# Orange-OpenSource/AIVC

Measured on AMD Instinct MI355X. Metric: encode+decode fps @1080p YUV420 (RA GOP32), higher is better.
Workload: dtype f32; 1 GPU; 1920x1080 8-bit YUV420, coding structure 1_GOP_32: one 128-frame clip = 4 intra-period units of 33 frames (132 coded frames, the last 4 repeat the last frame) encoded + decoded per step; synthetic random-init stand-in for model ms_ssim-4 (widths {'n2': 64, 'n': 128, 'c_y': 64, 'c_short': 64, 'c_z': 32, 'n_h': 128}), last analysis conv calibrated so that 6 (MOFNet) / 12 (CodecNet) of the 64 y featu; parallelism=single GPU

## Files before the change

aivc_amd/csrc/entropy.hip:

```cpp
#include <stdlib.h>
#include <string.h>

#include "common.h"

namespace aivc {

__device__ float balle_cdf_point(const float *P, float t) {
  const float *h0 = P, *h1 = P + 3, *h2 = P + 12, *h3 = P + 21;
  const float *b0 = P + 24, *b1 = P + 27, *b2 = P + 30, *b3 = P + 33;
  const float *a0 = P + 34, *a1 = P + 37, *a2 = P + 40;
  float v[3], nv[3];
#pragma unroll
  for (int r = 0; r < 3; ++r) {
    float x = t * aivc_softplusf_det(h0[r]);
    x = x + b0[r];
    v[r] = x + aivc_tanhf_det(a0[r]) * aivc_tanhf_det(x);
  }
#pragma unroll
  for (int l = 0; l < 2; ++l) {
    const float *hh = l == 0 ? h1 : h2;
    const float *bb = l == 0 ? b1 : b2;
    const float *aa = l == 0 ? a1 : a2;
#pragma unroll
    for (int r = 0; r < 3; ++r) {
      float acc = v[0] * aivc_softplusf_det(hh[0 * 3 + r]);
      acc = __builtin_fmaf(v[1], aivc_softplusf_det(hh[1 * 3 + r]), acc);
      acc = __builtin_fmaf(v[2], aivc_softplusf_det(hh[2 * 3 + r]), acc);
      const float x = acc + bb[r];
      nv[r] = x + aivc_tanhf_det(aa[r]) * aivc_tanhf_det(x);
    }
    v[0] = nv[0];
    v[1] = nv[1];
    v[2] = nv[2];
  }
  float acc = v[0] * aivc_softplusf_det(h3[0]);
  acc = __builtin_fmaf(v[1], aivc_softplusf_det(h3[1]), acc);
  acc = __builtin_fmaf(v[2], aivc_softplusf_det(h3[2]), acc);
  return aivc_sigmoidf_det(acc + b3[0]);
}

__global__ __launch_bounds__(256) void balle_cdf_table_kernel(const float *__restrict__ params, int c,
                                                              uint16_t *__restrict__ table,
                                                              float *__restrict__ cdf_f32) {
  const int gid = blockIdx.x * blockDim.x + threadIdx.x;
  if (gid >= c * AIVC_CDF_ROW) return;
  const int ch = gid / AIVC_CDF_ROW, k = gid % AIVC_CDF_ROW;
  if (k >= AIVC_LP) {
    table[gid] = 0;
    return;
  }
  const float cdf = balle_cdf_point(params + (size_t)ch * AIVC_BALLE_PARAMS, (float)k - 256.5f);
  if (cdf_f32) cdf_f32[(size_t)ch * AIVC_LP + k] = cdf;
  table[gid] = aivc_cdf_quant(cdf, k);
}

__global__ __launch_bounds__(256) void nonzero_maps_kernel(const int16_t *__restrict__ q, size_t npix, int c,
                                                           uint8_t *__restrict__ flags) {
  q += (size_t)blockIdx.y * npix * c;
  flags += (size_t)blockIdx.y * c;
  for (size_t i = (size_t)blockIdx.x * blockDim.x + threadIdx.x; i < npix * c; i += (size_t)gridDim.x * blockDim.x)
    if (q[i] != 0) flags[i % c] = 1;
}

__global__ __launch_bounds__(256) void laplace_cdf_rows_kernel(const float *__restrict__ sigma, size_t npix, int c,
                                                               aivc_map_list maps, uint16_t *__restrict__ rows) {
  constexpr int CHUNKS = AIVC_CDF_ROW / 8;
  const size_t gid = (size_t)blockIdx.x * blockDim.x + threadIdx.x;
  const size_t total = (size_t)maps.n_maps * npix * CHUNKS;
  if (gid >= total) return;
  const int chunk = (int)(gid % CHUNKS);
  const size_t pos = gid / CHUNKS;
  const int m = (int)(pos / npix);
  const size_t pix = pos % npix;
  const float s = sigma[pix * c + maps.idx[m]];
  uint32_t w[4];
#pragma unroll
  for (int j = 0; j < 4; ++j) {
    const int k0 = chunk * 8 + 2 * j, k1 = k0 + 1;
    const uint32_t lo = k0 < AIVC_LP ? aivc_laplace_cdf_u16(k0, s) : 0;
    const uint32_t hi = k1 < AIVC_LP ? aivc_laplace_cdf_u16(k1, s) : 0;
    w[j] = lo | (hi << 16);
  }
  *reinterpret_cast<uint4 *>(rows + pos * AIVC_CDF_ROW + chunk * 8) = make_uint4(w[0], w[1], w[2], w[3]);
}

using FrameTable = const aivc_frame_maps *__restrict__;
__device__ __forceinline__ const aivc_frame_maps &frame_of(FrameTable frames) { return frames[blockIdx.y]; }
__device__ __forceinline__ const aivc_frame_maps &frame_of(const aivc_frame_maps &fm) { return fm; }

constexpr int CDF_WIN0 = 224, CDF_WIN = 64;
template <class FRAMES>
__global__ __launch_bounds__(256) void laplace_cdf_windows_batch_kernel(const float *__restrict__ sigma, size_t npix, int c,
                                                                        const FRAMES frames, uint16_t *__restrict__ win,
                                                                        float *__restrict__ sigma_pos) {
  constexpr int CHUNKS = CDF_WIN / 8;
  const aivc_frame_maps &fm = frame_of(frames);
  const size_t gid = (size_t)blockIdx.x * blockDim.x + threadIdx.x;
  const size_t total = (size_t)fm.n_maps * npix;
  const size_t wv = gid >> 6;
  if ((wv / CHUNKS) * 64 >= total) return;
  const int lane = (int)(gid & 63), chunk = (int)(wv % CHUNKS);
  const size_t pos = (wv / CHUNKS) * 64 + (size_t)lane;
  const bool valid = pos < total;
  const float *sg = sigma + (size_t)blockIdx.y * npix * c;
  float s = 1.0f;
  if (valid) {
    const int m = (int)(pos / npix);
    const size_t pix = pos % npix;
    s = sg[pix * c + fm.idx[m]];
    if (chunk == 0) sigma_pos[fm.pos_off + pos] = s;
  }
  const int k0 = CDF_WIN0 + chunk * 8;
  uint32_t w[4];
  bool sat = false;
  if (chunk != CHUNKS / 2) {
    const float tmin = chunk < CHUNKS / 2 ? 256.5f - (float)(k0 + 7) : (float)k0 - 256.5f;
    const float b = s / 1.41421354f;
    sat = tmin / b > 17.5f;
  }
  if (__all(sat || !valid)) {
    const uint32_t base = chunk < CHUNKS / 2 ? 0u : 65023u;
#pragma unroll
    for (int j = 0; j < 4; ++j) {
      const uint32_t k = (uint32_t)(k0 + 2 * j);
      w[j] = ((base + k) & 0xFFFFu) | (((base + k + 1u) & 0xFFFFu) << 16);
    }
  } else {
#pragma unroll
    for (int j = 0; j < 4; ++j) {
      const int k = k0 + 2 * j;
      w[j] = (uint32_t)aivc_laplace_cdf_u16(k, s) | ((uint32_t)aivc_laplace_cdf_u16(k + 1, s) << 16);
    }
  }
  if (valid) *reinterpret_cast<uint4 *>(win + (fm.pos_off + pos) * CDF_WIN + chunk * 8) = make_uint4(w[0], w[1], w[2], w[3]);
}

template <class FRAMES>
__global__ __launch_bounds__(256) void laplace_bounds_batch_kernel(const float *__restrict__ sigma, const int16_t *__restrict__ q,
                                                                   size_t npix, int c, const FRAMES frames,
                                                                   uint32_t *__restrict__ bounds) {
  const aivc_frame_maps &fm = frame_of(frames);
  const size_t pos = (size_t)blockIdx.x * blockDim.x + threadIdx.x;
  if (pos >= (size_t)fm.n_maps * npix) return;
  const int ch = fm.idx[pos / npix];
  const size_t pix = pos % npix;
  const size_t o = ((size_t)blockIdx.y * npix + pix) * c + ch;
  const float s = sigma[o];
  const int sym = min(max((int)q[o] + AIVC_AC_MAX_VAL, 0), AIVC_MAX_SYMBOL);
  const uint32_t lo = aivc_laplace_cdf_u16(sym, s), hi = sym == AIVC_MAX_SYMBOL ? 0u : aivc_laplace_cdf_u16(sym + 1, s);
  bounds[fm.pos_off + pos] = lo | (hi << 16);
}

template <class FRAMES>
__global__ __launch_bounds__(256) void scatter_symbols_batch_kernel(const uint16_t *__restrict__ sym, size_t npix, int c,
                                                                    const FRAMES frames, int16_t *__restrict__ q, int vec) {
  __shared__ int16_t slot[AIVC_MAX_MAPS];
  const aivc_frame_maps &fm = frame_of(frames);
  for (int i = threadIdx.x; i < AIVC_MAX_MAPS; i += blockDim.x) slot[i] = -1;
  __syncthreads();
  for (int i = threadIdx.x; i < fm.n_maps; i += blockDim.x) slot[fm.idx[i]] = (int16_t)i;
  __syncthreads();
  const size_t gid = (size_t)blockIdx.x * blockDim.x + threadIdx.x;
  const int groups = (c + 7) / 8;
  if (gid >= npix * groups) return;
  const size_t pix = gid % npix;
  const int ch0 = (int)(gid / npix) * 8;
  const uint16_t *fs = sym + fm.pos_off;
  int16_t v[8];
#pragma unroll
  for (int e = 0; e < 8; ++e) {
    const int ch = ch0 + e;
    const int m = ch < c ? slot[ch] : -1;
    v[e] = m < 0 ? (int16_t)0 : (int16_t)((int)fs[(size_t)m * npix + pix] - AIVC_AC_MAX_VAL);
  }
  int16_t *dst = q + ((size_t)blockIdx.y * npix + pix) * c + ch0;
  if (vec) {
    uint4 o;
    o.x = (uint32_t)(uint16_t)v[0] | ((uint32_t)(uint16_t)v[1] << 16);
    o.y = (uint32_t)(uint16_t)v[2] | ((uint32_t)(uint16_t)v[3] << 16);
    o.z = (uint32_t)(uint16_t)v[4] | ((uint32_t)(uint16_t)v[5] << 16);
    o.w = (uint32_t)(uint16_t)v[6] | ((uint32_t)(uint16_t)v[7] << 16);
    *reinterpret_cast<uint4 *>(dst) = o;
  } else {
#pragma unroll
    for (int e = 0; e < 8; ++e)
      if (ch0 + e < c) dst[e] = v[e];
  }
}

__global__ __launch_bounds__(256) void table_bounds_batch_kernel(const uint16_t *__restrict__ table, const int16_t *__restrict__ q,
                                                                 size_t npix, int c, uint32_t *__restrict__ bounds) {
  const size_t pos = (size_t)blockIdx.x * blockDim.x + threadIdx.x;
  if (pos >= (size_t)c * npix) return;
  const int ch = (int)(pos / npix);
  const size_t pix = pos % npix;
  const int sym = min(max((int)q[((size_t)blockIdx.y * npix + pix) * c + ch] + AIVC_AC_MAX_VAL, 0), AIVC_MAX_SYMBOL);
  const uint16_t *row = table + (size_t)ch * AIVC_CDF_ROW;
  bounds[(size_t)blockIdx.y * c * npix + pos] = (uint32_t)row[sym] | (sym == AIVC_MAX_SYMBOL ? 0u : (uint32_t)row[sym + 1] << 16);
}

__device__ __forceinline__ uint32_t rl(uint32_t v, int lane) { return __builtin_amdgcn_readlane(v, lane); }

__device__ __forceinline__ uint32_t scaled(uint32_t e, uint32_t hl) {
  uint64_t r, carry;
  const uint64_t e64 = e;
  asm("v_mad_u64_u32 %0, %1, %2, %3, %4" : "=&v"(r), "=s"(carry) : "v"(e), "s"(hl), "v"(e64));
  uint32_t t = (uint32_t)(r >> 16);
  asm("" : "+v"(t));
  return t;
}

struct BitSink {
  uint32_t *out;
  uint32_t cap_words;
  uint32_t n_words;
  uint64_t acc;
  uint32_t nbits;
  uint32_t overflow;
  __device__ __forceinline__ void put(uint32_t bits, uint32_t nb) {
    acc = (acc << nb) | (uint64_t)bits;
    nbits += nb;
    if (nbits >= 32) {
      nbits -= 32;
      const uint32_t w = (uint32_t)(acc >> nbits);
      if (n_words < cap_words) out[n_words] = __builtin_bswap32(w);
      else overflow = 1;
      n_words++;
    }
  }
  __device__ __forceinline__ void put_run(uint32_t bit, uint32_t count) {
    while (count > 0) {
      const uint32_t r = count > 32 ? 32 : count;
      const uint32_t ones = r == 32 ? 0xFFFFFFFFu : ((1u << r) - 1u);
      put(bit ? ones : 0u, r);
      count -= r;
    }
  }
  __device__ __forceinline__ void finish() {
    if (nbits > 0) {
      const uint32_t w = (uint32_t)(acc << (32 - nbits));
      if (n_words < cap_words) out[n_words] = __builtin_bswap32(w);
      else overflow = 1;
    }
  }
};

__global__ __launch_bounds__(64) void range_encode_kernel(const uint32_t *__restrict__ bounds, aivc_rc_batch batch,
                                                          uint8_t *__restrict__ out, uint32_t *__restrict__ out_len) {
  const aivc_rc_stream st = batch.s[blockIdx.x];
  const int lane = threadIdx.x;
  __builtin_amdgcn_s_setprio(3);
  BitSink sink{reinterpret_cast<uint32_t *>(out + st.out_off), st.out_cap / 4, 0, 0, 0, 0};
  uint32_t low = 0, high = 0xFFFFFFFFu, pending = 0;
  const uint32_t *src = bounds + st.in_off;
  uint32_t nxt = lane < (int)st.n_sym ? src[lane] : 0u;
#pragma unroll 1
  for (uint32_t base = 0; base < st.n_sym; base += 64) {
    const uint32_t mine = nxt;
    nxt = (base + 64u + lane < st.n_sym) ? src[base + 64u + lane] : 0u;
    const uint32_t vlo = mine & 0xFFFFu, vhi = (mine >> 16) ? (mine >> 16) : 0x10000u;
    const uint32_t cnt = min(64u, st.n_sym - base);
#pragma unroll 1
    for (uint32_t j = 0; j < cnt; ++j) {
      const uint32_t hl = high - low;
      const uint32_t t_lo = rl(scaled(vlo, hl), (int)j), t_hi = rl(scaled(vhi, hl), (int)j);
      high = low + t_hi - 1u;
      low = low + t_lo;
      const uint32_t x = low ^ high;
      if ((int32_t)x >= 0) {
        const uint32_t n = (uint32_t)__builtin_clz(x | 1u);
        const uint32_t top = (uint32_t)(((uint64_t)low << n) >> 32);
        uint32_t bits = top, nb = n;
        if (pending != 0) {
          const uint32_t b0 = low >> 31;
          sink.put(b0, 1);
          sink.put_run(b0 ^ 1u, pending);
          pending = 0;
          nb = n - 1u;
          bits = top & ((1u << nb) - 1u);
        }
        sink.put(bits, nb);
        low <<= n;
        high = (high << n) | ~(0xFFFFFFFFu << n);
      }
      asm volatile("" : "+s"(high));
      const uint32_t yy = low & ~high;
      if (yy & 0x40000000u) {
        const uint32_t m = (uint32_t)__builtin_clz(~(yy << 1));
        pending += m;
        low = (low << m) & 0x7FFFFFFFu;
        high = (high << m) | 0x80000000u | ((1u << m) - 1u);
      }
    }
  }
  pending += 1;
  const uint32_t fb = low < 0x40000000u ? 0u : 1u;
  sink.put(fb, 1);
  sink.put_run(fb ^ 1u, pending);
  sink.finish();
  const uint32_t total = sink.n_words * 4u + (sink.nbits + 7u) / 8u;
  if (total > st.out_cap) sink.overflow = 1;
  if (lane == 0) out_len[blockIdx.x] = sink.overflow ? 0xFFFFFFFFu : total;
}

constexpr int ENC_CH = 32;

struct LanePacker {
  uint32_t *dst;
  uint32_t last_word;
  uint32_t widx;
  uint64_t acc;
  uint32_t nbits;
  __device__ __forceinline__ void push(uint32_t val, uint32_t len) {
    acc = (acc << len) | (uint64_t)val;
    nbits += len;
    dst[min(widx, last_word)] = __builtin_bswap32((uint32_t)(acc >> ((nbits - 32u) & 63u)));
    widx += nbits >> 5;
    nbits &= 31u;
  }
  __device__ __forceinline__ void put_run(uint32_t bit, uint32_t count) {
    while (count > 0) {
      const uint32_t r = count > 32 ? 32 : count;
      push(bit ? (r == 32 ? 0xFFFFFFFFu : ((1u << r) - 1u)) : 0u, r);
      count -= r;
    }
  }
  __device__ __forceinline__ void settle_long(uint32_t low, uint32_t n, uint32_t P) {
    if (n != 0) {
      const uint32_t b0 = low >> 31;
      push(b0, 1);
      put_run(b0 ^ 1u, P);
      push(((low << 1) >> 1) >> (32u - n), n - 1u);
    }
  }
};

__global__ __launch_bounds__(192) void range_encode_lanes_kernel(const uint32_t *__restrict__ bounds, aivc_rc_batch batch,
                                                                 uint8_t *__restrict__ out, uint32_t *__restrict__ out_len) {
  __shared__ uint32_t inb[2][ENC_CH][64];
  __shared__ uint2 rec[2][ENC_CH][64];
  __shared__ uint2 fin[64];
  const int lane = threadIdx.x & 63;
  const int wave = __builtin_amdgcn_readfirstlane((int)(threadIdx.x >> 6));
  const bool live = lane < batch.n_streams;
  const aivc_rc_stream st = batch.s[live ? lane : 0];
  const uint32_t n_sym = live ? st.n_sym : 0u;
  uint32_t n_max = n_sym;
#pragma unroll
  for (int off = 32; off > 0; off >>= 1) n_max = max(n_max, (uint32_t)__shfl_xor((int)n_max, off));
  n_max = __builtin_amdgcn_readfirstlane(n_max);
  const uint32_t n_chunks = (n_max + ENC_CH - 1) / ENC_CH;
  const uint32_t T = n_chunks + 2;
  __builtin_amdgcn_s_setprio(3);
  if (wave == 2) {
    const uint32_t *src = bounds + st.in_off;
    uint32_t r0[ENC_CH], r1[ENC_CH];
    auto fetch = [&](uint32_t (&r)[ENC_CH], uint32_t c) {
#pragma unroll
      for (int k = 0; k < ENC_CH; ++k) {
        const uint32_t i = c * ENC_CH + (uint32_t)k;
        r[k] = i < n_sym ? src[i] : 0u;
      }
    };
    auto stage = [&](const uint32_t (&r)[ENC_CH], uint32_t c) {
#pragma unroll
      for (int k = 0; k < ENC_CH; ++k) inb[c & 1][k][lane] = r[k];
    };
    fetch(r0, 0);
    fetch(r1, 1);
#pragma unroll 1
    for (uint32_t t = 0; t < T; t += 2) {
      if (t < n_chunks) {
        stage(r0, t);
        fetch(r0, t + 2);
      }
      __syncthreads();
      if (t + 1 < T) {
        if (t + 1 < n_chunks) {
          stage(r1, t + 1);
          fetch(r1, t + 3);
        }
        __syncthreads();
      }
    }
  } else if (wave == 0) {
    uint32_t low = 0, high = 0xFFFFFFFFu, pending = 0;
#pragma unroll 1
    for (uint32_t t = 0; t < T; ++t) {
      if (t >= 1 && t <= n_chunks) {
        const uint32_t c = t - 1;
        const uint32_t *ib = &inb[c & 1][0][lane];
        uint2 *buf = &rec[c & 1][0][lane];
#pragma unroll 8
        for (int k = 0; k < ENC_CH; ++k) {
          const uint32_t w = ib[k * 64];
          const uint32_t c_lo = w & 0xFFFFu;
          uint32_t c_hi = w >> 16;
          c_hi = c_hi ? c_hi : 0x10000u;
          const uint32_t hl = high - low;
          const uint32_t t_lo = (uint32_t)(((uint64_t)hl * c_lo + c_lo) >> 16);
          const uint32_t t_hi = (uint32_t)(((uint64_t)hl * c_hi + c_hi) >> 16);
          high = low + t_hi - 1u;
          low = low + t_lo;
          const uint32_t n = (uint32_t)__builtin_clz(low ^ high);
          const uint32_t P = n ? pending : 0u;
          pending = n ? 0u : pending;
          buf[k * 64] = make_uint2(low, n | (P << 5));
          const uint32_t yy = (low & ~high) << (n + 1u);
          const uint32_t m = (uint32_t)__builtin_clz(~yy);
          const uint32_t sh = n + m;
          pending += m;
          low = (low << sh) & 0x7FFFFFFFu;
          high = (high << sh) | ((1u << sh) - 1u) | 0x80000000u;
        }
      }
      if (t == n_chunks) fin[lane] = make_uint2(low, pending);
      __syncthreads();
    }
  } else {
    LanePacker pk{reinterpret_cast<uint32_t *>(out + st.out_off), st.out_cap / 4 - 1u, 0, 0, 0};
#pragma unroll 1
    for (uint32_t t = 0; t < T; ++t) {
      if (t >= 2 && live) {
        const uint32_t c = t - 2;
        const uint2 *buf = &rec[c & 1][0][lane];
        const LanePacker at_start = pk;
        uint32_t longest = 0;
#pragma unroll 8
        for (int k = 0; k < ENC_CH; ++k) {
          const uint2 r = buf[k * 64];
          const uint32_t low = r.x, n = r.y & 31u, P = r.y >> 5;
          const uint32_t len = n + P;
          longest = max(longest, len);
          const uint32_t n1 = n ? n - 1u : 0u;
          const uint32_t head = ((1u << P) - 1u) + (low >> 31);
          const uint32_t rest = ((low << 1) >> 1) >> (31u - n1);
          uint32_t val = (head << n1) | rest;
          asm volatile("" : "+v"(val));
          pk.push(n ? val : 0u, len);
        }
        if (__builtin_expect(__ballot(longest > 32u) != 0ull, 0)) {
          pk = at_start;
#pragma unroll 1
          for (int k = 0; k < ENC_CH; ++k) {
            const uint2 r = buf[k * 64];
            pk.settle_long(r.x, r.y & 31u, r.y >> 5);
          }
        }
      }
      __syncthreads();
    }
    const uint2 f = fin[lane];
    if (live) {
      const uint32_t fb = f.x < 0x40000000u ? 0u : 1u;
      pk.push(fb, 1);
      pk.put_run(fb ^ 1u, f.y + 1u);
      if (pk.nbits > 0) pk.dst[min(pk.widx, pk.last_word)] = __builtin_bswap32((uint32_t)(pk.acc << (32 - pk.nbits)));
      const uint32_t total = pk.widx * 4u + (pk.nbits + 7u) / 8u;
      out_len[lane] = total > st.out_cap ? 0xFFFFFFFFu : total;
    }
  }
}

struct BitWin {
  const uint32_t *in;
  uint32_t n_words;
  uint32_t tail_bytes;
  uint32_t wi;
  uint32_t chunk;
  uint64_t win;
  uint32_t avail;
  int lane;
  __device__ __forceinline__ void load_chunk() {
    const uint32_t idx = (wi & ~63u) + (uint32_t)lane;
    uint32_t w = idx < n_words ? in[idx] : 0u;
    if (idx + 1 == n_words && tail_bytes) w &= (1u << (8 * tail_bytes)) - 1u;
    chunk = w;
  }
  __device__ __forceinline__ uint32_t next_word() {
    const uint32_t w = __builtin_bswap32(rl(chunk, (int)(wi & 63u)));
    wi++;
    if ((wi & 63u) == 0) load_chunk();
    return w;
  }
  __device__ __forceinline__ void init() {
    wi = 0;
    load_chunk();
    win = (uint64_t)next_word() << 32;
    win |= (uint64_t)next_word();
    avail = 64;
  }
  __device__ __forceinline__ uint32_t value() const { return (uint32_t)(win >> 32); }
  __device__ __forceinline__ void consume(uint32_t n) {
    win <<= n;
    avail -= n;
    if (__builtin_expect(avail <= 32, 0)) {
      win |= (uint64_t)next_word() << (32 - avail);
      avail += 32;
    }
  }
};

constexpr int DEC_HALF = 32;
constexpr int DEC_SLOTS = 2 * DEC_HALF + 1;
constexpr int DEC_WIN0 = 224;
static_assert(DEC_WIN0 == CDF_WIN0, "window position");

__device__ __forceinline__ void window_dma(const uint16_t *base, uint32_t voff, uint32_t lds_dst) {
  asm volatile("s_mov_b32 m0, %2\n\ts_nop 0\n\tglobal_load_lds_ushort %0, %1" : : "v"(voff), "s"(base), "s"(lds_dst) : "memory", "m0");
}

template <bool PLANE, bool WINDOWED = false>
__device__ __forceinline__ uint32_t decode_stream(const uint8_t *__restrict__ bytes, const uint16_t *__restrict__ rows,
                                              const aivc_rc_stream &st, uint16_t *__restrict__ sym, uint32_t *ring,
                                              const int lane, const float *sigma_ring = nullptr) {
  static_assert(!(PLANE && WINDOWED), "windows are per-position Laplace rows");
  constexpr int ROWLEN = WINDOWED ? CDF_WIN : AIVC_CDF_ROW;
  constexpr int WOFF = WINDOWED ? 0 : DEC_WIN0;
  BitWin bw;
  bw.in = reinterpret_cast<const uint32_t *>(bytes + st.in_off);
  bw.n_words = (st.in_len + 3u) / 4u;
  bw.tail_bytes = st.in_len & 3u;
  bw.lane = lane;
  bw.init();
  uint32_t low = 0, high = 0xFFFFFFFFu;
  const uint32_t n_sym = st.n_sym, plane = st.plane;
  const uint16_t *base = rows + st.row_off * ROWLEN;
  auto row_of = [&](uint32_t i) -> const uint16_t * { return base + (uint64_t)(PLANE ? i / plane : i) * ROWLEN; };
  uint32_t ew_next = 0;

  uint32_t mysym = 0;
#pragma unroll 1
  for (uint32_t first = 0; first < n_sym; first += (uint32_t)DEC_HALF) {
    const uint32_t cnt = min((uint32_t)DEC_HALF, n_sym - first);
    __syncthreads();
    const uint32_t *hw = ring + ((first / DEC_HALF) & 1u) * (DEC_HALF * 64) + lane;
    ew_next = hw[0];
    auto finish = [&](const uint32_t j, const uint32_t m, const uint32_t t_lo, const uint32_t t_hi) __attribute__((always_inline)) {
      mysym = (uint32_t)lane == ((first + j) & 63u) ? m : mysym;
      high = low + t_hi - 1u;
      low = low + t_lo;
      const uint32_t x = low ^ high;
      const uint32_t yy = (low & ~high) << 1;
      if ((yy | ~x) & 0x80000000u) {
        const uint32_t n = (uint32_t)__builtin_clz(x);
        const uint32_t m3 = (uint32_t)__builtin_clz(~(yy << n));
        const uint32_t sh = n + m3;
        low = (low << sh) & 0x7FFFFFFFu;
        high = (high << sh) | ((1u << sh) - 1u) | 0x80000000u;
        bw.consume(sh);
        bw.win ^= (uint64_t)(m3 != 0u) << 63;
      }
    };
    auto step = [&](const uint32_t j) __attribute__((always_inline)) {
      const uint32_t ew = ew_next;
      ew_next = hw[(j + 1u) * 64u];
      const uint32_t hl = high - low;
      const uint32_t d = bw.value() - low;
      uint32_t m, t_lo, t_hi;
      const uint32_t tw = scaled(ew, hl);
      const uint32_t cw = (uint32_t)__builtin_popcountll(__ballot(tw <= d));
      m = (uint32_t)DEC_WIN0 - 1u + cw;
      t_lo = rl(tw, (int)cw - 1);
      t_hi = rl(tw, (int)cw);
      if (__builtin_expect(cw - 1u >= 63u, 0)) {
        uint32_t i = first + j;
        asm volatile("" : "+s"(i));
        if constexpr (WINDOWED) {
          const float sg = sigma_ring[((first / DEC_HALF) & 1u) * DEC_HALF + j];
          if (cw == 0u) {
            uint32_t above = rl(tw, 0);
            int base = DEC_WIN0 - 64;
#pragma unroll 1
            for (;;) {
              const uint32_t tf = scaled((uint32_t)aivc_laplace_cdf_u16_scale(base + lane, sg), hl);
              uint32_t c = (uint32_t)__builtin_popcountll(__ballot(tf <= d));
              if (base == 0) c = max(c, 1u);
              if (c > 0u) {
                m = (uint32_t)base + c - 1u;
                t_lo = rl(tf, (int)c - 1);
                t_hi = c < 64u ? rl(tf, (int)c) : above;
                break;
              }
              above = rl(tf, 0);
              base = base >= 64 ? base - 64 : 0;
            }
          } else {
            uint32_t below = rl(tw, 63);
            int base = DEC_WIN0 + 64;
#pragma unroll 1
            for (;;) {
              const int k = base + lane;
              const uint32_t tf = scaled((uint32_t)aivc_laplace_cdf_u16_scale(min(k, AIVC_MAX_SYMBOL), sg), hl);
              const uint32_t c = (uint32_t)__builtin_popcountll(__ballot(k < AIVC_MAX_SYMBOL && tf <= d));
              if (c < 64u) {
                m = (uint32_t)base + c - 1u;
                t_lo = c > 0u ? rl(tf, (int)c - 1) : below;
                t_hi = rl(tf, (int)c);
                break;
              }
              below = rl(tf, 63);
              base += 64;
            }
          }
        } else {
          uint32_t t[9];
          const uint16_t *row = row_of(i);
          const uint4 e = *reinterpret_cast<const uint4 *>(row + lane * 8);
          const uint32_t nx = row[lane * 8 + 8];
          t[0] = scaled(e.x & 0xFFFFu, hl); t[1] = scaled(e.x >> 16, hl);
          t[2] = scaled(e.y & 0xFFFFu, hl); t[3] = scaled(e.y >> 16, hl);
          t[4] = scaled(e.z & 0xFFFFu, hl); t[5] = scaled(e.z >> 16, hl);
          t[6] = scaled(e.w & 0xFFFFu, hl); t[7] = scaled(e.w >> 16, hl);
          t[8] = scaled(nx, hl);
          uint32_t total = 0;
#pragma unroll
          for (int k = 0; k < 8; ++k) total += (uint32_t)__builtin_popcountll(__ballot(t[k] <= d));
          m = total > 0 ? total - 1 : 0;
          const int L = (int)(m >> 3);
          const uint32_t idx = m & 7u;
          uint32_t s_lo = t[0], s_hi = t[1];
#pragma unroll
          for (int k = 1; k < 8; ++k) {
            s_lo = idx == (uint32_t)k ? t[k] : s_lo;
            s_hi = idx == (uint32_t)k ? t[k + 1] : s_hi;
          }
          t_lo = rl(s_lo, L);
          t_hi = rl(s_hi, L);
        }
        if (m == 511u && t_hi <= d) {
          m = 512u;
          t_lo = t_hi;
          t_hi = hl + 1u;
        }
      }
      finish(j, m, t_lo, t_hi);
    };
    uint32_t j = 0;
#pragma unroll 1
    for (; j + 4u <= cnt; j += 4u) {
      step(j);
      step(j + 1u);
      step(j + 2u);
      step(j + 3u);
    }
#pragma unroll 1
    for (; j < cnt; ++j) step(j);
    const uint32_t g0 = first & ~63u, done = first + cnt;
    if (((done & 63u) == 0u || done == n_sym) && (uint32_t)lane < done - g0) sym[st.out_off + g0 + lane] = (uint16_t)mysym;
  }
  return bw.wi * 32u - bw.avail;
}

template <bool PLANE, bool WINDOWED = false>
__device__ __forceinline__ void decode_prefetcher(const uint16_t *__restrict__ rows, const aivc_rc_stream &st, uint32_t *ring,
                                                  const int lane, const float *__restrict__ sigma_pos = nullptr,
                                                  float *sigma_ring = nullptr) {
  constexpr int ROWLEN = WINDOWED ? CDF_WIN : AIVC_CDF_ROW;
  constexpr int WOFF = WINDOWED ? 0 : DEC_WIN0;
  const uint32_t ring_base = (uint32_t)(uintptr_t)(__attribute__((address_space(3))) uint32_t *)ring;
  const uint32_t n_sym = st.n_sym, plane = st.plane;
  const uint32_t n_rows = PLANE ? (n_sym + plane - 1u) / plane : n_sym;
  const uint16_t *base = rows + st.row_off * ROWLEN;
  uint32_t voff = (uint32_t)(WOFF + lane) * 2u;
  const uint32_t vlast = voff + (n_rows - 1u) * (uint32_t)(ROWLEN * 2);
  uint32_t in_plane = 0;
#pragma unroll 1
  for (uint32_t first = 0; first < n_sym; first += (uint32_t)DEC_HALF) {
    const uint32_t half = ring_base + ((first / DEC_HALF) & 1u) * (DEC_HALF * 256);
    float sg = 1.f;
    if constexpr (WINDOWED)
      sg = sigma_pos[st.row_off + min(first + (uint32_t)(lane & (DEC_HALF - 1)), n_sym - 1u)];
#pragma unroll 8
    for (uint32_t k = 0; k < (uint32_t)DEC_HALF; ++k) {
      window_dma(base, voff, half + k * 256u);
      uint32_t step = (uint32_t)(ROWLEN * 2);
      if (PLANE) {
        ++in_plane;
        const bool wrap = in_plane == plane;
        step = wrap ? step : 0u;
        in_plane = wrap ? 0u : in_plane;
      }
      voff = min(voff + step, vlast);
    }
    asm volatile("s_waitcnt vmcnt(0)" ::: "memory");
    if constexpr (WINDOWED)
      if (lane < DEC_HALF) sigma_ring[((first / DEC_HALF) & 1u) * DEC_HALF + lane] = aivc_laplace_scale(sg);
    __syncthreads();
  }
}

__global__ __launch_bounds__(128) void range_decode_kernel(const uint8_t *__restrict__ bytes,
                                                           const uint16_t *__restrict__ rows, aivc_rc_batch batch,
                                                           uint16_t *__restrict__ sym, uint32_t *__restrict__ consumed) {
  __shared__ uint32_t ring[DEC_SLOTS * 64];
  const aivc_rc_stream st = batch.s[blockIdx.x];
  const int lane = threadIdx.x & 63;
  const int wave = __builtin_amdgcn_readfirstlane((int)(threadIdx.x >> 6));
  if (st.n_sym == 0) {
    if (consumed && threadIdx.x == 0) consumed[blockIdx.x] = 0;
    return;
  }
  __builtin_amdgcn_s_setprio(3);
  if (wave == 1) {
    if (st.plane) decode_prefetcher<true>(rows, st, ring, lane);
    else decode_prefetcher<false>(rows, st, ring, lane);
    return;
  }
  uint32_t bits;
  if (st.plane) bits = decode_stream<true>(bytes, rows, st, sym, ring, lane);
  else bits = decode_stream<false>(bytes, rows, st, sym, ring, lane);
  if (consumed && lane == 0) consumed[blockIdx.x] = bits;
}

__global__ __launch_bounds__(128) void range_decode_windows_kernel(const uint8_t *__restrict__ bytes,
                                                                   const uint16_t *__restrict__ win,
                                                                   const float *__restrict__ sigma_pos, aivc_rc_batch batch,
                                                                   uint16_t *__restrict__ sym, uint32_t *__restrict__ consumed) {
  __shared__ uint32_t ring[DEC_SLOTS * 64];
  __shared__ float sigma_ring[2 * DEC_HALF];
  const aivc_rc_stream st = batch.s[blockIdx.x];
  const int lane = threadIdx.x & 63;
  const int wave = __builtin_amdgcn_readfirstlane((int)(threadIdx.x >> 6));
  if (st.n_sym == 0) {
    if (consumed && threadIdx.x == 0) consumed[blockIdx.x] = 0;
    return;
  }
  __builtin_amdgcn_s_setprio(3);
  if (wave == 1) {
    decode_prefetcher<false, true>(win, st, ring, lane, sigma_pos, sigma_ring);
    return;
  }
  const uint32_t bits = decode_stream<false, true>(bytes, win, st, sym, ring, lane, sigma_ring);
  if (consumed && lane == 0) consumed[blockIdx.x] = bits;
}

}

using namespace aivc;

AIVC_EXPORT int aivc_balle_cdf_table(const float *params, int32_t c, uint16_t *table, float *cdf_f32,
                                     aivc_stream_t stream) {
  if (!params || !table || c <= 0) return AIVC_ERR_ARG;
  hipLaunchKernelGGL(balle_cdf_table_kernel, dim3(cdiv((size_t)c * AIVC_CDF_ROW, 256)), dim3(256), 0,
                     to_stream(stream), params, c, table, cdf_f32);
  return check_launch("balle_cdf_table");
}

AIVC_EXPORT int aivc_nonzero_maps_batch(const int16_t *q, int32_t n, size_t npix, int32_t c, uint8_t *flags,
                                        aivc_stream_t stream) {
  if (!q || !flags || c <= 0 || c > AIVC_MAX_MAPS || n <= 0 || n > 65535) return AIVC_ERR_ARG;
  if (hipMemsetAsync(flags, 0, (size_t)n * c, to_stream(stream)) != hipSuccess) return check_launch("nonzero_maps memset");
  if (npix == 0) return AIVC_OK;
  unsigned grid = cdiv(npix * c, 256 * 8);
  grid = grid > 2048 ? 2048 : (grid == 0 ? 1 : grid);
  hipLaunchKernelGGL(nonzero_maps_kernel, dim3(grid, (unsigned)n), dim3(256), 0, to_stream(stream), q, npix, c, flags);
  return check_launch("nonzero_maps");
}

AIVC_EXPORT int aivc_nonzero_maps(const int16_t *q, size_t npix, int32_t c, uint8_t *flags, aivc_stream_t stream) {
  return aivc_nonzero_maps_batch(q, 1, npix, c, flags, stream);
}

static int check_maps(const aivc_map_list *maps, int c) {
  if (!maps || maps->n_maps < 0 || maps->n_maps > c || c > AIVC_MAX_MAPS) return AIVC_ERR_ARG;
  for (int i = 0; i < maps->n_maps; ++i)
    if (maps->idx[i] >= c) return AIVC_ERR_ARG;
  return AIVC_OK;
}

static aivc_frame_maps one_frame(const aivc_map_list *maps) {
  aivc_frame_maps fm = {};
  fm.n_maps = maps->n_maps;
  memcpy(fm.idx, maps->idx, sizeof fm.idx);
  return fm;
}

AIVC_EXPORT int aivc_laplace_cdf_rows(const float *sigma, size_t npix, int32_t c, const aivc_map_list *maps,
                                      uint16_t *rows, aivc_stream_t stream) {
  if (!sigma || !rows || c <= 0) return AIVC_ERR_ARG;
  if (int rc = check_maps(maps, c)) return rc;
  const size_t total = (size_t)maps->n_maps * npix * (AIVC_CDF_ROW / 8);
  if (total == 0) return AIVC_OK;
  hipLaunchKernelGGL(laplace_cdf_rows_kernel, dim3(cdiv(total, 256)), dim3(256), 0, to_stream(stream), sigma, npix,
                     c, *maps, rows);
  return check_launch("laplace_cdf_rows");
}

AIVC_EXPORT int aivc_laplace_bounds(const float *sigma, const int16_t *q, size_t npix, int32_t c,
                                    const aivc_map_list *maps, uint32_t *bounds, aivc_stream_t stream) {
  if (!sigma || !q || !bounds || c <= 0) return AIVC_ERR_ARG;
  if (int rc = check_maps(maps, c)) return rc;
  const size_t total = (size_t)maps->n_maps * npix;
  if (total == 0) return AIVC_OK;
  hipLaunchKernelGGL(laplace_bounds_batch_kernel<aivc_frame_maps>, dim3(cdiv(total, 256)), dim3(256), 0, to_stream(stream),
                     sigma, q, npix, c, one_frame(maps), bounds);
  return check_launch("laplace_bounds");
}

AIVC_EXPORT int aivc_table_bounds(const uint16_t *table, const int16_t *q, size_t npix, int32_t c, uint32_t *bounds,
                                  aivc_stream_t stream) {
  return aivc_table_bounds_batch(table, q, 1, npix, c, bounds, stream);
}

AIVC_EXPORT int aivc_scatter_symbols(const uint16_t *sym, size_t npix, int32_t c, const aivc_map_list *maps,
                                     int16_t *q, aivc_stream_t stream) {
  if (!q || c <= 0) return AIVC_ERR_ARG;
  if (int rc = check_maps(maps, c)) return rc;
  if (maps->n_maps > 0 && !sym) return AIVC_ERR_ARG;
  if (npix == 0) return AIVC_OK;
  const int vec = (c & 7) == 0 && ((uintptr_t)q & 15) == 0;
  hipLaunchKernelGGL(scatter_symbols_batch_kernel<aivc_frame_maps>, dim3(cdiv(npix * ((c + 7) / 8), 256)), dim3(256), 0,
                     to_stream(stream), sym, npix, c, one_frame(maps), q, vec);
  return check_launch("scatter_symbols");
}

AIVC_EXPORT int aivc_laplace_cdf_windows_batch(const float *sigma, int32_t n, size_t npix, int32_t c,
                                               const aivc_frame_maps *frames, int32_t max_maps, uint16_t *win,
                                               float *sigma_pos, aivc_stream_t stream) {
  if (!sigma || !frames || !win || !sigma_pos || c <= 0 || c > AIVC_MAX_MAPS || n <= 0 || n > 65535 || max_maps < 0 || max_maps > c)
    return AIVC_ERR_ARG;
  const size_t n_pos = (size_t)max_maps * npix;
  if (n_pos == 0) return AIVC_OK;
  const size_t total = ((n_pos + 63) / 64) * (CDF_WIN / 8) * 64;
  hipLaunchKernelGGL(laplace_cdf_windows_batch_kernel<FrameTable>, dim3(cdiv(total, 256), (unsigned)n), dim3(256), 0, to_stream(stream),
                     sigma, npix, c, frames, win, sigma_pos);
  return check_launch("laplace_cdf_windows_batch");
}

AIVC_EXPORT int aivc_laplace_bounds_batch(const float *sigma, const int16_t *q, int32_t n, size_t npix, int32_t c,
                                          const aivc_frame_maps *frames, int32_t max_maps, uint32_t *bounds,
                                          aivc_stream_t stream) {
  if (!sigma || !q || !frames || !bounds || c <= 0 || c > AIVC_MAX_MAPS || n <= 0 || n > 65535 || max_maps < 0 || max_maps > c)
    return AIVC_ERR_ARG;
  const size_t total = (size_t)max_maps * npix;
  if (total == 0) return AIVC_OK;
  hipLaunchKernelGGL(laplace_bounds_batch_kernel<FrameTable>, dim3(cdiv(total, 256), (unsigned)n), dim3(256), 0, to_stream(stream), sigma, q,
                     npix, c, frames, bounds);
  return check_launch("laplace_bounds_batch");
}

AIVC_EXPORT int aivc_table_bounds_batch(const uint16_t *table, const int16_t *q, int32_t n, size_t npix, int32_t c,
                                        uint32_t *bounds, aivc_stream_t stream) {
  if (!table || !q || !bounds || c <= 0 || n <= 0 || n > 65535) return AIVC_ERR_ARG;
  if (npix == 0) return AIVC_OK;
  hipLaunchKernelGGL(table_bounds_batch_kernel, dim3(cdiv((size_t)c * npix, 256), (unsigned)n), dim3(256), 0, to_stream(stream),
                     table, q, npix, c, bounds);
  return check_launch("table_bounds_batch");
}

AIVC_EXPORT int aivc_scatter_symbols_batch(const uint16_t *sym, int32_t n, size_t npix, int32_t c,
                                           const aivc_frame_maps *frames, int16_t *q, aivc_stream_t stream) {
  if (!q || !frames || !sym || c <= 0 || c > AIVC_MAX_MAPS || n <= 0 || n > 65535) return AIVC_ERR_ARG;
  if (npix == 0) return AIVC_OK;
  const int vec = (c & 7) == 0 && ((uintptr_t)q & 15) == 0;
  hipLaunchKernelGGL(scatter_symbols_batch_kernel<FrameTable>, dim3(cdiv(npix * ((c + 7) / 8), 256), (unsigned)n), dim3(256), 0,
                     to_stream(stream), sym, npix, c, frames, q, vec);
  return check_launch("scatter_symbols_batch");
}

static int check_batch(const aivc_rc_batch *b) {
  if (!b || b->n_streams < 0 || b->n_streams > AIVC_RC_MAX_STREAMS) return AIVC_ERR_ARG;
  return AIVC_OK;
}

AIVC_EXPORT int aivc_range_encode(const uint32_t *bounds, const aivc_rc_batch *batch, uint8_t *out,
                                  uint32_t *out_len, aivc_stream_t stream) {
  if (!out || !out_len) return AIVC_ERR_ARG;
  if (int rc = check_batch(batch)) return rc;
  if (batch->n_streams == 0) return AIVC_OK;
  for (int i = 0; i < batch->n_streams; ++i) {
    if (batch->s[i].out_off % 4) return AIVC_ERR_ARG;
    if (batch->s[i].out_cap < 4 || batch->s[i].out_cap % 4) return AIVC_ERR_ARG;
    if (batch->s[i].n_sym && !bounds) return AIVC_ERR_ARG;
  }
  const char *mode = getenv("AIVC_RC_ENCODE");
  if (mode && !strcmp(mode, "wave"))
    hipLaunchKernelGGL(range_encode_kernel, dim3(batch->n_streams), dim3(64), 0, to_stream(stream), bounds, *batch, out, out_len);
  else {
    static const int own_cu = getenv("AIVC_RC_OWN_CU") ? atoi(getenv("AIVC_RC_OWN_CU")) : 1;
    uint32_t longest = 0;
    for (int i = 0; i < batch->n_streams; ++i) longest = batch->s[i].n_sym > longest ? batch->s[i].n_sym : longest;
    size_t pad_lds = 0;
    if (own_cu && longest >= 65536u) {
      static LdsOptIn opt_in;
      pad_lds = 100 * 1024;
      if (!opt_in.raise(reinterpret_cast<const void *>(range_encode_lanes_kernel), pad_lds)) pad_lds = 0;
    }
    hipLaunchKernelGGL(range_encode_lanes_kernel, dim3(1), dim3(192), pad_lds, to_stream(stream), bounds, *batch, out, out_len);
  }
  return check_launch("range_encode");
}

AIVC_EXPORT int aivc_laplace_cdf_windows(const float *sigma, size_t npix, int32_t c, const aivc_map_list *maps,
                                         uint16_t *win, float *sigma_pos, aivc_stream_t stream) {
  if (!sigma || !win || !sigma_pos || c <= 0) return AIVC_ERR_ARG;
  if (int rc = check_maps(maps, c)) return rc;
  const size_t n_pos = (size_t)maps->n_maps * npix;
  if (n_pos == 0) return AIVC_OK;
  const size_t total = ((n_pos + 63) / 64) * (CDF_WIN / 8) * 64;
  hipLaunchKernelGGL(laplace_cdf_windows_batch_kernel<aivc_frame_maps>, dim3(cdiv(total, 256)), dim3(256), 0, to_stream(stream),
                     sigma, npix, c, one_frame(maps), win, sigma_pos);
  return check_launch("laplace_cdf_windows");
}

AIVC_EXPORT int aivc_range_decode_windows(const uint8_t *bytes, const uint16_t *win, const float *sigma_pos,
                                          const aivc_rc_batch *batch, uint16_t *sym, uint32_t *consumed_bits,
                                          aivc_stream_t stream) {
  if (!bytes || !win || !sigma_pos || !sym) return AIVC_ERR_ARG;
  if (int rc = check_batch(batch)) return rc;
  if (batch->n_streams == 0) return AIVC_OK;
  for (int i = 0; i < batch->n_streams; ++i) {
    if (batch->s[i].in_off % 4 || batch->s[i].plane != 0) return AIVC_ERR_ARG;
    if (((uint64_t)batch->s[i].n_sym + 1) * (uint64_t)(CDF_WIN * 2) >= 0x100000000ull) return AIVC_ERR_UNSUPPORTED;
  }
  hipLaunchKernelGGL(range_decode_windows_kernel, dim3(batch->n_streams), dim3(128), 0, to_stream(stream), bytes, win,
                     sigma_pos, *batch, sym, consumed_bits);
  return check_launch("range_decode_windows");
}

AIVC_EXPORT int aivc_range_decode(const uint8_t *bytes, const uint16_t *rows, const aivc_rc_batch *batch,
                                  uint16_t *sym, uint32_t *consumed_bits, aivc_stream_t stream) {
  if (!bytes || !rows || !sym) return AIVC_ERR_ARG;
  if (int rc = check_batch(batch)) return rc;
  if (batch->n_streams == 0) return AIVC_OK;
  for (int i = 0; i < batch->n_streams; ++i) {
    if (batch->s[i].in_off % 4) return AIVC_ERR_ARG;
    const uint64_t n_rows = batch->s[i].plane ? (batch->s[i].n_sym + batch->s[i].plane - 1) / batch->s[i].plane : batch->s[i].n_sym;
    if ((n_rows + 1) * (uint64_t)(AIVC_CDF_ROW * 2) >= 0x100000000ull) return AIVC_ERR_UNSUPPORTED;
  }
  hipLaunchKernelGGL(range_decode_kernel, dim3(batch->n_streams), dim3(128), 0, to_stream(stream), bytes, rows,
                     *batch, sym, consumed_bits);
  return check_launch("range_decode");
}
```

Baseline: 103.0 frames/s.

## Pack four decode streams per workgroup with LDS counter handshakes instead of barriers

Range decoding previously used one 128-thread workgroup per stream, with decoder and prefetcher waves synchronised by __syncthreads. Now each workgroup holds four decoder/prefetcher wave pairs, each with its own LDS ring, and each pair synchronises through produced/consumed counters using atomic loads, release stores and s_sleep polling. The aim is to cut workgroup count and dispatch cost and to let pairs run independently without block-wide barriers. The cost is reserved dynamic LDS, optionally padded to own a CU for long streams, plus spin-wait overhead and a risk of ordering bugs in the handshake.

```diff
diff --git a/aivc_amd/csrc/decode_groups.h b/aivc_amd/csrc/decode_groups.h
--- /dev/null
+++ b/aivc_amd/csrc/decode_groups.h
@@ -0,0 +1,43 @@
+#pragma once
+#include <stdint.h>
+
+#if defined(__HIPCC__) || defined(__CUDACC__)
+#define AIVC_DEC_GROUPS_HD __host__ __device__
+#else
+#define AIVC_DEC_GROUPS_HD
+#endif
+
+namespace aivc {
+
+constexpr uint32_t DEC_GROUP = 4u;
+
+constexpr uint32_t DEC_HALF = 32u;
+constexpr uint32_t DEC_SLOTS = 2u * DEC_HALF + 1u;
+
+constexpr uint32_t DEC_LDS_RING = 0u;
+constexpr uint32_t DEC_LDS_SIGMA = DEC_SLOTS * 64u * 4u;
+constexpr uint32_t DEC_LDS_PRODUCED = DEC_LDS_SIGMA + 2u * DEC_HALF * 4u;
+constexpr uint32_t DEC_LDS_CONSUMED = DEC_LDS_PRODUCED + 4u;
+constexpr uint32_t DEC_LDS_PAIR = DEC_LDS_CONSUMED + 12u;
+
+constexpr uint32_t DEC_CU_LDS = 160u * 1024u;
+constexpr uint32_t DEC_OWNED_LDS = 148u * 1024u + 512u;
+constexpr uint32_t DEC_OWN_CU_SYMBOLS = 65536u;
+
+AIVC_DEC_GROUPS_HD constexpr uint32_t dec_grid(uint32_t n_streams, uint32_t g) { return (n_streams + g - 1u) / g; }
+AIVC_DEC_GROUPS_HD constexpr uint32_t dec_lds_own(uint32_t g) { return g * DEC_LDS_PAIR; }
+AIVC_DEC_GROUPS_HD constexpr uint32_t dec_lds_pad(uint32_t g) { return dec_lds_own(g) < DEC_OWNED_LDS ? DEC_OWNED_LDS - dec_lds_own(g) : 0u; }
+AIVC_DEC_GROUPS_HD constexpr uint32_t dec_lds_pair(uint32_t pair) { return pair * DEC_LDS_PAIR; }
+
+struct DecRole {
+  uint32_t pair;
+  bool prefetcher;
+};
+AIVC_DEC_GROUPS_HD constexpr DecRole dec_wave_role(uint32_t wave, uint32_t g) { return {wave < g ? wave : wave - g, wave >= g}; }
+AIVC_DEC_GROUPS_HD constexpr uint32_t dec_stream_of(uint32_t wg, uint32_t pair, uint32_t g) { return wg * g + pair; }
+
+AIVC_DEC_GROUPS_HD constexpr bool dec_may_fill(uint32_t b, uint32_t consumed) { return b < consumed + 2u; }
+AIVC_DEC_GROUPS_HD constexpr bool dec_may_read(uint32_t b, uint32_t produced) { return b < produced; }
+AIVC_DEC_GROUPS_HD constexpr uint32_t dec_halves(uint32_t n_sym) { return (n_sym + DEC_HALF - 1u) / DEC_HALF; }
+
+}
diff --git a/aivc_amd/csrc/entropy.hip b/aivc_amd/csrc/entropy.hip
--- a/aivc_amd/csrc/entropy.hip
+++ b/aivc_amd/csrc/entropy.hip
@@ -2,6 +2,7 @@
 #include <string.h>
 
 #include "common.h"
+#include "decode_groups.h"
 
 namespace aivc {
 
@@ -501,19 +502,36 @@
   }
 };
 
-constexpr int DEC_HALF = 32;
-constexpr int DEC_SLOTS = 2 * DEC_HALF + 1;
 constexpr int DEC_WIN0 = 224;
 static_assert(DEC_WIN0 == CDF_WIN0, "window position");
 
 __device__ __forceinline__ void window_dma(const uint16_t *base, uint32_t voff, uint32_t lds_dst) {
   asm volatile("s_mov_b32 m0, %2\n\ts_nop 0\n\tglobal_load_lds_ushort %0, %1" : : "v"(voff), "s"(base), "s"(lds_dst) : "memory", "m0");
+}
+
+__device__ __forceinline__ uint32_t dec_look(const uint32_t *counter) {
+  return __hip_atomic_load(counter, __ATOMIC_RELAXED, __HIP_MEMORY_SCOPE_WORKGROUP);
+}
+template <bool FILL>
+__device__ __forceinline__ void dec_wait(const uint32_t *counter, const uint32_t b, const uint32_t seen) {
+  uint32_t c = (uint32_t)__builtin_amdgcn_readfirstlane((int)seen);
+  if (__builtin_expect(!(FILL ? dec_may_fill(b, c) : dec_may_read(b, c)), 0)) {
+    do {
+      __builtin_amdgcn_s_sleep(1);
+      c = (uint32_t)__builtin_amdgcn_readfirstlane((int)dec_look(counter));
+    } while (!(FILL ? dec_may_fill(b, c) : dec_may_read(b, c)));
+  }
+  asm volatile("" ::: "memory");
+}
+__device__ __forceinline__ void dec_publish(uint32_t *counter, const uint32_t halves, const int lane) {
+  if (lane == 0) __hip_atomic_store(counter, halves, __ATOMIC_RELEASE, __HIP_MEMORY_SCOPE_WORKGROUP);
 }
 
 template <bool PLANE, bool WINDOWED = false>
 __device__ __forceinline__ uint32_t decode_stream(const uint8_t *__restrict__ bytes, const uint16_t *__restrict__ rows,
                                               const aivc_rc_stream &st, uint16_t *__restrict__ sym, uint32_t *ring,
-                                              const int lane, const float *sigma_ring = nullptr) {
+                                              uint32_t *produced, uint32_t *consumed, const int lane,
+                                              const float *sigma_ring = nullptr) {
   static_assert(!(PLANE && WINDOWED), "windows are per-position Laplace rows");
   constexpr int ROWLEN = WINDOWED ? CDF_WIN : AIVC_CDF_ROW;
   constexpr int WOFF = WINDOWED ? 0 : DEC_WIN0;
@@ -530,10 +548,11 @@
   uint32_t ew_next = 0;
 
   uint32_t mysym = 0;
+  uint32_t seen = dec_look(produced);
 #pragma unroll 1
   for (uint32_t first = 0; first < n_sym; first += (uint32_t)DEC_HALF) {
     const uint32_t cnt = min((uint32_t)DEC_HALF, n_sym - first);
-    __syncthreads();
+    dec_wait<false>(produced, first / DEC_HALF, seen);
     const uint32_t *hw = ring + ((first / DEC_HALF) & 1u) * (DEC_HALF * 64) + lane;
     ew_next = hw[0];
     auto finish = [&](const uint32_t j, const uint32_t m, const uint32_t t_lo, const uint32_t t_hi) __attribute__((always_inline)) {
@@ -647,14 +666,17 @@
 #pragma unroll 1
     for (; j < cnt; ++j) step(j);
     const uint32_t g0 = first & ~63u, done = first + cnt;
+    seen = dec_look(produced);
     if (((done & 63u) == 0u || done == n_sym) && (uint32_t)lane < done - g0) sym[st.out_off + g0 + lane] = (uint16_t)mysym;
+    dec_publish(consumed, first / DEC_HALF + 1u, lane);
   }
   return bw.wi * 32u - bw.avail;
 }
 
 template <bool PLANE, bool WINDOWED = false>
 __device__ __forceinline__ void decode_prefetcher(const uint16_t *__restrict__ rows, const aivc_rc_stream &st, uint32_t *ring,
-                                                  const int lane, const float *__restrict__ sigma_pos = nullptr,
+                                                  uint32_t *produced, const uint32_t *consumed, const int lane,
+                                                  const float *__restrict__ sigma_pos = nullptr,
                                                   float *sigma_ring = nullptr) {
   constexpr int ROWLEN = WINDOWED ? CDF_WIN : AIVC_CDF_ROW;
   constexpr int WOFF = WINDOWED ? 0 : DEC_WIN0;
@@ -668,6 +690,7 @@
 #pragma unroll 1
   for (uint32_t first = 0; first < n_sym; first += (uint32_t)DEC_HALF) {
     const uint32_t half = ring_base + ((first / DEC_HALF) & 1u) * (DEC_HALF * 256);
+    dec_wait<true>(consumed, first / DEC_HALF, dec_look(consumed));
     float sg = 1.f;
     if constexpr (WINDOWED)
       sg = sigma_pos[st.row_off + min(first + (uint32_t)(lane & (DEC_HALF - 1)), n_sym - 1u)];
@@ -685,54 +708,75 @@
     }
     asm volatile("s_waitcnt vmcnt(0)" ::: "memory");
     if constexpr (WINDOWED)
-      if (lane < DEC_HALF) sigma_ring[((first / DEC_HALF) & 1u) * DEC_HALF + lane] = aivc_laplace_scale(sg);
-    __syncthreads();
-  }
-}
-
-__global__ __launch_bounds__(128) void range_decode_kernel(const uint8_t *__restrict__ bytes,
-                                                           const uint16_t *__restrict__ rows, aivc_rc_batch batch,
-                                                           uint16_t *__restrict__ sym, uint32_t *__restrict__ consumed) {
-  __shared__ uint32_t ring[DEC_SLOTS * 64];
-  const aivc_rc_stream st = batch.s[blockIdx.x];
+      if ((uint32_t)lane < DEC_HALF) sigma_ring[((first / DEC_HALF) & 1u) * DEC_HALF + lane] = aivc_laplace_scale(sg);
+    dec_publish(produced, first / DEC_HALF + 1u, lane);
+  }
+}
+
+struct DecPair {
+  uint32_t stream;
+  bool prefetcher;
+  uint32_t *ring, *produced, *consumed;
+  float *sigma_ring;
+};
+template <int G>
+__device__ __forceinline__ DecPair dec_pair_of_wave(uint8_t *lds) {
+  const DecRole role = dec_wave_role((uint32_t)__builtin_amdgcn_readfirstlane((int)(threadIdx.x >> 6)), (uint32_t)G);
+  uint8_t *mine = lds + dec_lds_pair(role.pair);
+  DecPair p = {dec_stream_of(blockIdx.x, role.pair, (uint32_t)G), role.prefetcher, reinterpret_cast<uint32_t *>(mine + DEC_LDS_RING),
+               reinterpret_cast<uint32_t *>(mine + DEC_LDS_PRODUCED), reinterpret_cast<uint32_t *>(mine + DEC_LDS_CONSUMED),
+               reinterpret_cast<float *>(mine + DEC_LDS_SIGMA)};
+  if (!role.prefetcher && (threadIdx.x & 63) == 0) *p.produced = *p.consumed = 0u;
+  __syncthreads();
+  return p;
+}
+
+template <int G>
+__global__ __launch_bounds__(128 * G) void range_decode_kernel(const uint8_t *__restrict__ bytes,
+                                                               const uint16_t *__restrict__ rows, aivc_rc_batch batch,
+                                                               uint16_t *__restrict__ sym, uint32_t *__restrict__ consumed) {
+  extern __shared__ __attribute__((aligned(16))) uint8_t dec_lds[];
+  const DecPair p = dec_pair_of_wave<G>(dec_lds);
+  if (p.stream >= (uint32_t)batch.n_streams) return;
+  const aivc_rc_stream st = batch.s[p.stream];
   const int lane = threadIdx.x & 63;
-  const int wave = __builtin_amdgcn_readfirstlane((int)(threadIdx.x >> 6));
   if (st.n_sym == 0) {
-    if (consumed && threadIdx.x == 0) consumed[blockIdx.x] = 0;
+    if (consumed && !p.prefetcher && lane == 0) consumed[p.stream] = 0;
     return;
   }
   __builtin_amdgcn_s_setprio(3);
-  if (wave == 1) {
-    if (st.plane) decode_prefetcher<true>(rows, st, ring, lane);
-    else decode_prefetcher<false>(rows, st, ring, lane);
+  if (p.prefetcher) {
+    if (st.plane) decode_prefetcher<true>(rows, st, p.ring, p.produced, p.consumed, lane);
+    else decode_prefetcher<false>(rows, st, p.ring, p.produced, p.consumed, lane);
     return;
   }
   uint32_t bits;
-  if (st.plane) bits = decode_stream<true>(bytes, rows, st, sym, ring, lane);
-  else bits = decode_stream<false>(bytes, rows, st, sym, ring, lane);
-  if (consumed && lane == 0) consumed[blockIdx.x] = bits;
-}
-
-__global__ __launch_bounds__(128) void range_decode_windows_kernel(const uint8_t *__restrict__ bytes,
-                                                                   const uint16_t *__restrict__ win,
-                                                                   const float *__restrict__ sigma_pos, aivc_rc_batch batch,
-                                                                   uint16_t *__restrict__ sym, uint32_t *__restrict__ consumed) {
-  __shared__ uint32_t ring[DEC_SLOTS * 64];
-  __shared__ float sigma_ring[2 * DEC_HALF];
-  const aivc_rc_stream st = batch.s[blockIdx.x];
+  if (st.plane) bits = decode_stream<true>(bytes, rows, st, sym, p.ring, p.produced, p.consumed, lane);
+  else bits = decode_stream<false>(bytes, rows, st, sym, p.ring, p.produced, p.consumed, lane);
+  if (consumed && lane == 0) consumed[p.stream] = bits;
+}
+
+template <int G>
+__global__ __launch_bounds__(128 * G) void range_decode_windows_kernel(const uint8_t *__restrict__ bytes,
+                                                                       const uint16_t *__restrict__ win,
+                                                                       const float *__restrict__ sigma_pos, aivc_rc_batch batch,
+                                                                       uint16_t *__restrict__ sym, uint32_t *__restrict__ consumed) {
+  extern __shared__ __attribute__((aligned(16))) uint8_t dec_lds[];
+  const DecPair p = dec_pair_of_wave<G>(dec_lds);
+  if (p.stream >= (uint32_t)batch.n_streams) return;
+  const aivc_rc_stream st = batch.s[p.stream];
   const int lane = threadIdx.x & 63;
-  const int wave = __builtin_amdgcn_readfirstlane((int)(threadIdx.x >> 6));
   if (st.n_sym == 0) {
-    if (consumed && threadIdx.x == 0) consumed[blockIdx.x] = 0;
+    if (consumed && !p.prefetcher && lane == 0) consumed[p.stream] = 0;
     return;
   }
   __builtin_amdgcn_s_setprio(3);
-  if (wave == 1) {
-    decode_prefetcher<false, true>(win, st, ring, lane, sigma_pos, sigma_ring);
+  if (p.prefetcher) {
+    decode_prefetcher<false, true>(win, st, p.ring, p.produced, p.consumed, lane, sigma_pos, p.sigma_ring);
     return;
   }
-  const uint32_t bits = decode_stream<false, true>(bytes, win, st, sym, ring, lane, sigma_ring);
-  if (consumed && lane == 0) consumed[blockIdx.x] = bits;
+  const uint32_t bits = decode_stream<false, true>(bytes, win, st, sym, p.ring, p.produced, p.consumed, lane, p.sigma_ring);
+  if (consumed && lane == 0) consumed[p.stream] = bits;
 }
 
 }
@@ -892,6 +936,16 @@
   return check_launch("range_encode");
 }
 
+static bool decode_lds(const void *kernel, LdsOptIn &opt_in, const aivc_rc_batch *batch, size_t *lds) {
+  static const int own_cu = getenv("AIVC_RC_OWN_CU") ? atoi(getenv("AIVC_RC_OWN_CU")) : 1;
+  static_assert(dec_lds_own(DEC_GROUP) + dec_lds_pad(DEC_GROUP) <= DEC_CU_LDS, "a decoding workgroup fits a CU");
+  if (!opt_in.raise(kernel, DEC_CU_LDS)) return false;
+  uint32_t longest = 0;
+  for (int i = 0; i < batch->n_streams; ++i) longest = batch->s[i].n_sym > longest ? batch->s[i].n_sym : longest;
+  *lds = dec_lds_own(DEC_GROUP) + (own_cu && longest >= DEC_OWN_CU_SYMBOLS ? dec_lds_pad(DEC_GROUP) : 0u);
+  return true;
+}
+
 AIVC_EXPORT int aivc_laplace_cdf_windows(const float *sigma, size_t npix, int32_t c, const aivc_map_list *maps,
                                          uint16_t *win, float *sigma_pos, aivc_stream_t stream) {
   if (!sigma || !win || !sigma_pos || c <= 0) return AIVC_ERR_ARG;
@@ -914,8 +968,14 @@
     if (batch->s[i].in_off % 4 || batch->s[i].plane != 0) return AIVC_ERR_ARG;
     if (((uint64_t)batch->s[i].n_sym + 1) * (uint64_t)(CDF_WIN * 2) >= 0x100000000ull) return AIVC_ERR_UNSUPPORTED;
   }
-  hipLaunchKernelGGL(range_decode_windows_kernel, dim3(batch->n_streams), dim3(128), 0, to_stream(stream), bytes, win,
-                     sigma_pos, *batch, sym, consumed_bits);
+  size_t lds = 0;
+  static LdsOptIn opt_in;
+  if (!decode_lds(reinterpret_cast<const void *>(range_decode_windows_kernel<(int)DEC_GROUP>), opt_in, batch, &lds)) {
+    (void)check_launch("range_decode lds attribute");
+    return AIVC_ERR_LAUNCH;
+  }
+  hipLaunchKernelGGL(range_decode_windows_kernel<(int)DEC_GROUP>, dim3(dec_grid((uint32_t)batch->n_streams, DEC_GROUP)), dim3(128 * DEC_GROUP), lds,
+                     to_stream(stream), bytes, win, sigma_pos, *batch, sym, consumed_bits);
   return check_launch("range_decode_windows");
 }
 
@@ -929,7 +989,13 @@
     const uint64_t n_rows = batch->s[i].plane ? (batch->s[i].n_sym + batch->s[i].plane - 1) / batch->s[i].plane : batch->s[i].n_sym;
     if ((n_rows + 1) * (uint64_t)(AIVC_CDF_ROW * 2) >= 0x100000000ull) return AIVC_ERR_UNSUPPORTED;
   }
-  hipLaunchKernelGGL(range_decode_kernel, dim3(batch->n_streams), dim3(128), 0, to_stream(stream), bytes, rows,
-                     *batch, sym, consumed_bits);
+  size_t lds = 0;
+  static LdsOptIn opt_in;
+  if (!decode_lds(reinterpret_cast<const void *>(range_decode_kernel<(int)DEC_GROUP>), opt_in, batch, &lds)) {
+    (void)check_launch("range_decode lds attribute");
+    return AIVC_ERR_LAUNCH;
+  }
+  hipLaunchKernelGGL(range_decode_kernel<(int)DEC_GROUP>, dim3(dec_grid((uint32_t)batch->n_streams, DEC_GROUP)), dim3(128 * DEC_GROUP), lds,
+                     to_stream(stream), bytes, rows, *batch, sym, consumed_bits);
   return check_launch("range_decode");
 }
```

Result: no change. 103.5 frames/s, median of 6 (+0.5%).
